# google/tfp-causalimpact

Measured on AMD Instinct MI355X. Metric: posterior samples/sec (T=1000, 10 covariates), higher is better.
Workload: dtype f32; 1 GPU; cfg2: T=1000, 10 covariates (P=11), LocalLinearTrend + spike-and-slab regression, Gibbs, W=112, S=1000; sampler=gibbs, chains_per_gpu=8, chains_total=8, parallelism=chains sharded over 1 GPU(s), no data-path collective, launcher=single process, collectives=none, ranks_seen=1

## Files before the change

tfp-causalimpact_amd/csrc/ci_kernels.h:

```cpp
#pragma once
#include <hip/hip_runtime.h>
#include <type_traits>
#include <stdint.h>

#include "ci_linalg.h"
#include "ci_rng.h"

namespace ci {

constexpr int NT = 256;
constexpr int NW = 4;
constexpr int MAXP = 52;
constexpr int HMC_MAXP = 128;

struct DevSeriesParams {
  double level_conc, level_scale, level_ub;
  double slope_conc, slope_scale, slope_ub;
  double obs_conc, obs_scale, obs_ub;
  double nonzero_prob;
  double init_level_loc, init_level_scale, init_slope_scale;
  double obs_scale0, level_scale0, slope_scale0;
  double n_obs;
};

struct KArgs {
  int T, P, W, S, C, B, chain_offset;
  int series_stream_base;
  uint32_t seed0, seed1;
  int x_in_lds;
  const float* y;
  const uint8_t* mask;
  const float* Xt;
  const double* xtx;
  const double* omega;
  const DevSeriesParams* sp;
  float* out_obs;
  float* out_level_scale;
  float* out_slope_scale;
  float* out_weights;
  float* out_level;
  float* out_slope;
  float* out_pred_mean;
  float* out_traj;
  long long* prof;
  unsigned int* progress;
  int progress_every;
  int dbg;
  const int* series_T;
  const int* series_ids;
};

__host__ __device__ inline uint32_t stream_mix32(uint32_t h) {
  h ^= h >> 16; h *= 0x85EBCA6Bu; h ^= h >> 13; h *= 0xC2B2AE35u; h ^= h >> 16;
  return h;
}
__host__ __device__ inline uint32_t stream_sid(int series_stream_base, int series) {
  return series_stream_base < 0 ? 0u : (uint32_t)(series_stream_base + series);
}
__host__ __device__ inline uint32_t stream_key0(uint32_t seed0, int series_stream_base, int series) {
  return seed0 ^ stream_mix32(stream_sid(series_stream_base, series));
}
__host__ __device__ inline uint32_t stream_key1(uint32_t seed1, int series_stream_base, int series) {
  return seed1 ^ stream_mix32(stream_sid(series_stream_base, series) * 0x9E3779B9u);
}

__device__ __forceinline__ void wave_sync() {
  __builtin_amdgcn_fence(__ATOMIC_SEQ_CST, "workgroup");
  __builtin_amdgcn_wave_barrier();
}

struct Prof {
  long long* p;
  long long t;
  __device__ __forceinline__ void start(long long* ptr, bool active) {
    p = active ? ptr : nullptr;
    if (p) t = clock64();
  }
  __device__ __forceinline__ void tick(int slot) {
    if (p) {
      const long long n = clock64();
      p[slot] += n - t;
      t = n;
    }
  }
};

struct NoProf {
  __device__ __forceinline__ void start(long long*, bool) {}
  __device__ __forceinline__ void tick(int) {}
};

template <class E> struct Arr { float f[sizeof(E) / 4]; };

template <class E> __device__ __forceinline__ E shfl_up_e(const E& e, int off) {
  Arr<E> a = __builtin_bit_cast(Arr<E>, e);
#pragma unroll
  for (int i = 0; i < (int)(sizeof(E) / 4); ++i) a.f[i] = __shfl_up(a.f[i], off, 64);
  return __builtin_bit_cast(E, a);
}
template <class E> __device__ __forceinline__ E shfl_down_e(const E& e, int off) {
  Arr<E> a = __builtin_bit_cast(Arr<E>, e);
#pragma unroll
  for (int i = 0; i < (int)(sizeof(E) / 4); ++i) a.f[i] = __shfl_down(a.f[i], off, 64);
  return __builtin_bit_cast(E, a);
}
template <class E> __device__ __forceinline__ void lds_store_e(float* p, const E& e) {
  const Arr<E> a = __builtin_bit_cast(Arr<E>, e);
#pragma unroll
  for (int i = 0; i < (int)(sizeof(E) / 4); ++i) p[i] = a.f[i];
}
template <class E> __device__ __forceinline__ E lds_load_e(const float* p) {
  Arr<E> a;
#pragma unroll
  for (int i = 0; i < (int)(sizeof(E) / 4); ++i) a.f[i] = p[i];
  return __builtin_bit_cast(E, a);
}

template <int CTRL, int ROW_MASK, class E> __device__ __forceinline__ E dpp_move_e(const E& e) {
  Arr<E> a = __builtin_bit_cast(Arr<E>, e);
#pragma unroll
  for (int i = 0; i < (int)(sizeof(E) / 4); ++i)
    a.f[i] = __int_as_float(__builtin_amdgcn_update_dpp(__float_as_int(a.f[i]), __float_as_int(a.f[i]),
                                                        CTRL, ROW_MASK, 0xF, false));
  return __builtin_bit_cast(E, a);
}
template <int CTRL, int ROW_MASK, class E> __device__ __forceinline__ E dpp_take_e(const E& e) {
  Arr<E> a = __builtin_bit_cast(Arr<E>, e);
#pragma unroll
  for (int i = 0; i < (int)(sizeof(E) / 4); ++i)
    a.f[i] = __int_as_float(__builtin_amdgcn_mov_dpp(__float_as_int(a.f[i]), CTRL, ROW_MASK, 0xF, true));
  return __builtin_bit_cast(E, a);
}
template <class E> __device__ __forceinline__ E select_e(bool c, const E& a, const E& b) {
  Arr<E> x = __builtin_bit_cast(Arr<E>, a);
  const Arr<E> y = __builtin_bit_cast(Arr<E>, b);
#pragma unroll
  for (int i = 0; i < (int)(sizeof(E) / 4); ++i) x.f[i] = c ? x.f[i] : y.f[i];
  return __builtin_bit_cast(E, x);
}

template <class E, class Op>
__device__ __forceinline__ E wave_scan_incl_fwd(const E& v, Op op, int lane) {
  E incl = v;
  const int r = lane & 15;
  { const E o = dpp_take_e<0x111, 0xF>(incl); if (r >= 1) incl = op(o, incl); }
  { const E o = dpp_take_e<0x112, 0xF>(incl); if (r >= 2) incl = op(o, incl); }
  { const E o = dpp_take_e<0x114, 0xF>(incl); if (r >= 4) incl = op(o, incl); }
  { const E o = dpp_take_e<0x118, 0xF>(incl); if (r >= 8) incl = op(o, incl); }
  { const E o = dpp_take_e<0x142, 0xA>(incl); if (lane & 16) incl = op(o, incl); }
  { const E o = dpp_take_e<0x143, 0xC>(incl); if (lane & 32) incl = op(o, incl); }
  return incl;
}
template <class E, class Op>
__device__ __forceinline__ E wave_scan_incl_bwd(const E& v, Op op, int lane) {
  E incl = v;
  const int r = lane & 15;
  { const E o = dpp_take_e<0x101, 0xF>(incl); if (r < 15) incl = op(incl, o); }
  { const E o = dpp_take_e<0x102, 0xF>(incl); if (r < 14) incl = op(incl, o); }
  { const E o = dpp_take_e<0x104, 0xF>(incl); if (r < 12) incl = op(incl, o); }
  { const E o = dpp_take_e<0x108, 0xF>(incl); if (r < 8) incl = op(incl, o); }
  {
    const Arr<E> b = __builtin_bit_cast(Arr<E>, dpp_take_e<0x150, 0xF>(incl));
    Arr<E> a;
#pragma unroll
    for (int i = 0; i < (int)(sizeof(E) / 4); ++i) {
      const auto s = __builtin_amdgcn_permlane16_swap((unsigned)__float_as_int(b.f[i]), 0u, false, false);
      a.f[i] = __int_as_float((int)s[1]);
    }
    const E o = __builtin_bit_cast(E, a);
    if ((lane & 16) == 0) incl = op(incl, o);
  }
  {
    Arr<E> a = __builtin_bit_cast(Arr<E>, incl);
#pragma unroll
    for (int i = 0; i < (int)(sizeof(E) / 4); ++i)
      a.f[i] = __int_as_float(__builtin_amdgcn_readlane(__float_as_int(a.f[i]), 32));
    const E o = __builtin_bit_cast(E, a);
    if ((lane & 32) == 0) incl = op(incl, o);
  }
  return incl;
}

template <class E, class Op>
__device__ __forceinline__ E block_scan_fwd_begin(const E& tot, Op op, float* slots, int lane, int wave) {
  constexpr int N = sizeof(E) / 4;
  const E incl = wave_scan_incl_fwd(tot, op, lane);
  if (lane == 63) lds_store_e(slots + wave * N, incl);
  return incl;
}
template <class E, class Op>
__device__ __forceinline__ E block_scan_fwd_finish(const E& incl, Op op, const E& ident, const float* slots,
                                                   int lane, int wave) {
  constexpr int N = sizeof(E) / 4;
  const E ex = select_e(lane == 0, ident, dpp_take_e<0x138, 0xF>(incl));
  if (wave == 0) return ex;
  E wp = lds_load_e<E>(slots);
  for (int ww = 1; ww < wave; ++ww) wp = op(wp, lds_load_e<E>(slots + ww * N));
  return op(wp, ex);
}
template <class E, class Op>
__device__ __forceinline__ E block_scan_excl_fwd(const E& tot, Op op, const E& ident, float* slots,
                                                 int lane, int wave) {
  const E incl = block_scan_fwd_begin(tot, op, slots, lane, wave);
  __syncthreads();
  return block_scan_fwd_finish(incl, op, ident, slots, lane, wave);
}

template <class E, class Op>
__device__ __forceinline__ E block_scan_excl_bwd(const E& tot, Op op, const E& ident, float* slots,
                                                 int lane, int wave) {
  constexpr int N = sizeof(E) / 4;
  const E incl = wave_scan_incl_bwd(tot, op, lane);
  if (lane == 0) lds_store_e(slots + wave * N, incl);
  __syncthreads();
  const E ex = select_e(lane == 63, ident, dpp_take_e<0x130, 0xF>(incl));
  if (wave == NW - 1) return ex;
  E ws = lds_load_e<E>(slots + (wave + 1) * N);
  for (int ww = wave + 2; ww < NW; ++ww) ws = op(ws, lds_load_e<E>(slots + ww * N));
  return op(ex, ws);
}

template <int L>
__device__ __forceinline__ void global_row_load_wide(const float* __restrict__ row, int t0, int T,
                                                     float (&v)[L]) {
  static_assert(L % 4 == 0, "wide rows need L % 4 == 0");
#pragma unroll
  for (int q = 0; q < L / 4; ++q) {
    const int t = t0 + 4 * q;
    const float4 x = *reinterpret_cast<const float4*>(row + (t < T ? t : T - 4));
    const bool in = t < T;
    v[4 * q] = in ? x.x : 0.f; v[4 * q + 1] = in ? x.y : 0.f;
    v[4 * q + 2] = in ? x.z : 0.f; v[4 * q + 3] = in ? x.w : 0.f;
  }
}
template <int L>
__device__ __forceinline__ void global_row_load_scalar(const float* __restrict__ row, int t0, int T,
                                                       float (&v)[L]) {
#pragma unroll
  for (int l = 0; l < L; ++l) {
    const int t = t0 + l;
    const float x = row[t < T ? t : T - 1];
    v[l] = t < T ? x : 0.f;
// ... 3079 lines not shown
```

tfp-causalimpact_amd/csrc/ci_kernels8.h:

```cpp
#pragma once
#include "ci_kernels.h"

namespace ci {

constexpr int SCHED_DEFAULT = (2 << 4) | (1 << 6) | (0 << 8) | (2 << 10) | (2 << 12) | (0 << 14);
constexpr int NT8 = 512;
constexpr int NW8 = 8;
constexpr int PRE_MAXS = 16;

struct PreTables {
  double* tsw;
  double* V;
  double* rdk;
  double* hand;
};
constexpr size_t PRE_HALF_DOUBLES = PRE_MAXS * 16 + 16 * 16 + 16;
__host__ __device__ constexpr size_t pre_tables_bytes() {
  return sizeof(double) * (2 * PRE_HALF_DOUBLES + 20) + 16;
}
__device__ __forceinline__ PreTables pre_tables_at(unsigned char* base, int parity) {
  PreTables tb;
  double* d = (double*)base + (size_t)(parity & 1) * PRE_HALF_DOUBLES;
  tb.tsw = d; d += PRE_MAXS * 16;
  tb.V = d; d += 16 * 16;
  tb.rdk = d;
  tb.hand = (double*)base + 2 * PRE_HALF_DOUBLES;
  return tb;
}
constexpr int HAND_SCALE = 16, HAND_INTS = 17;

struct PreState {
  double c[4];
  double diag;
  double rdk;
  unsigned long long S;
  int n_sw;
  int valid;
};

template <int CTRL> __device__ __forceinline__ double dpp_ror_add_d(double v) {
  const int lo = __builtin_amdgcn_update_dpp(0, __double2loint(v), CTRL, 0xF, 0xF, false);
  const int hi = __builtin_amdgcn_update_dpp(0, __double2hiint(v), CTRL, 0xF, 0xF, false);
  return v + __hiloint2double(hi, lo);
}
__device__ __forceinline__ double row_sum16_d(double v) {
  v = dpp_ror_add_d<0x128>(v);
  v = dpp_ror_add_d<0x124>(v);
  v = dpp_ror_add_d<0x122>(v);
  v = dpp_ror_add_d<0x121>(v);
  return readlane_d(v, 0);
}

template <int KR>
__device__ __forceinline__ void sweep_rec_kr(QCols& m, int k, int lane, double& t_out, double& rd_out) {
  const int kq = k >> 2, j = lane & 15, q = lane >> 4;
  const double ckr = m.c[KR];
  const double rd = fast_rcp(readlane_d(ckr, k + 16 * kq));
  const double rowk = bperm_d(ckr, j + 16 * kq);
  const bool isk = j == k;
  const double t = isk ? 1.0 : rowk * rd;
  double colk[4];
#pragma unroll
  for (int r = 0; r < 4; ++r) colk[r] = bperm_d(m.c[r], k + 16 * q);
  __builtin_amdgcn_sched_barrier(0);
#pragma unroll
  for (int r = 0; r < 4; ++r) m.c[r] = isk ? colk[r] * rd : m.c[r] - colk[r] * t;
  m.c[KR] = (q == kq) ? (isk ? -rd : t) : m.c[KR];
  m.diag = isk ? -rd : m.diag - rowk * rowk * rd;
  t_out = t;
  rd_out = rd;
}
__device__ __forceinline__ void sweep_rec(QCols& m, int k, int lane, double& t_out, double& rd_out) {
  switch (k & 3) {
    case 0: sweep_rec_kr<0>(m, k, lane, t_out, rd_out); break;
    case 1: sweep_rec_kr<1>(m, k, lane, t_out, rd_out); break;
    case 2: sweep_rec_kr<2>(m, k, lane, t_out, rd_out); break;
    default: sweep_rec_kr<3>(m, k, lane, t_out, rd_out); break;
  }
}

struct PreRun {
  QCols m;
  double rdk;
  unsigned long long pending;
  int n;
  int phase;
};
__device__ __forceinline__ void pre_begin(PreRun& st, unsigned long long S) {
  st.pending = S;
  st.n = 0;
  st.rdk = 0.0;
  st.phase = 0;
}
__device__ __forceinline__ void pre_step(PreRun& st, const RegLds& R, int P, double var_next,
                                         unsigned long long S, int lane, const PreTables& tb,
                                         PreState& ps) {
  const int j = lane & 15, q = lane >> 4;
  const bool live = j < P;
  const int col = live ? j : 0;
  if (st.phase == 0) {
#pragma unroll
    for (int r = 0; r < 4; ++r) {
      const int i = 4 * q + r;
      double om = 0.0, xx = 0.0;
      if (live && i < P) {
        om = R.omega[i * P + col];
        xx = R.xtx[i * P + col];
      }
      st.m.c[r] = om * var_next + xx;
      st.m.p[r] = 0.0;
    }
    st.m.diag = live ? R.omega[col * P + col] * var_next + R.xtx[col * P + col] : 1.0;
    st.m.cb = 0.0; st.m.corner = 0.0; st.m.pdiag = 0.0;
    st.phase = st.pending != 0ull ? 1 : 2;
  } else if (st.phase == 1) {
    const int k = __builtin_amdgcn_readfirstlane(__ffsll((long long)st.pending) - 1);
    double t, rd;
    sweep_rec(st.m, k, lane, t, rd);
    if (q == 0) tb.tsw[st.n * 16 + j] = t;
    st.rdk = (j == k) ? rd : st.rdk;
    ++st.n;
    st.pending &= st.pending - 1ull;
    if (st.pending == 0ull) st.phase = 2;
  } else {
#pragma unroll
    for (int r = 0; r < 4; ++r) tb.V[(4 * q + r) * 16 + j] = st.m.c[r];
    if (q == 0) tb.rdk[j] = st.rdk;
    ps.n_sw = st.n;
#pragma unroll
    for (int r = 0; r < 4; ++r) ps.c[r] = st.m.c[r];
    ps.diag = st.m.diag;
    ps.rdk = st.rdk;
    ps.S = S;
    ps.valid = 1;
    st.phase = 3;
  }
}

__device__ __forceinline__ void weights_backsub(const PreTables& tb, const double* pre, int P,
                                                unsigned long long S, double mean, double new_scale,
                                                int lane, float* w) {
  const int j = lane & 15, q = lane >> 4;
  const bool live = j < P;
  const float zf = reinterpret_cast<const float*>(pre + 24)[live ? j : 0];
  const bool inS = ((S >> j) & 1ull) != 0ull;
  const int pos = __popcll(S & ((1ull << j) - 1ull));
  const int n_sw = __popcll(S);
  const double rsz = (double)__fsqrt_rn((float)tb.rdk[j]) * (double)zf;
  double tt[PRE_MAXS];
#pragma unroll
  for (int s = 0; s < PRE_MAXS; ++s) tt[s] = tb.tsw[s * 16 + j];
  double u = 0.0;
#pragma unroll
  for (int s = PRE_MAXS - 1; s >= 0; --s) {
    if (s < n_sw) {
      double dot = (inS && pos > s) ? tt[s] * u : 0.0;
      dot = dpp_ror_add_d<0x128>(dot);
      dot = dpp_ror_add_d<0x124>(dot);
      dot = dpp_ror_add_d<0x122>(dot);
      dot = dpp_ror_add_d<0x121>(dot);
      u = (inS && pos == s) ? rsz - dot : u;
    }
  }
  if (q == 0 && live) w[j] = inS ? (float)(mean + new_scale * u) : 0.f;
}

template <class PF, class Pub>
__device__ __forceinline__ double spike_slab_draw_pre(const RegLds& R, int P,
                                                      const DevSeriesParams& sp,
                                                      double prev_obs_scale, double g_obs,
                                                      int lane, PriorCarry& pc, const double* pre,
                                                      const PreTables& tb, const PreState& ps,
                                                      const float* red, PF& prof, Pub publish) {
  const double prev_var = prev_obs_scale * prev_obs_scale;
  const double a_post = sp.obs_conc + 0.5 * sp.n_obs;
  const bool all_in = sp.nonzero_prob >= 1.0;
  const int j = lane & 15, q = lane >> 4;
  const bool live = j < P;
  const int col = live ? j : 0;
  QCols m;
#pragma unroll
  for (int r = 0; r < 4; ++r) { m.c[r] = ps.c[r]; m.p[r] = pc.p[r]; }
  m.diag = ps.diag;
  m.pdiag = pc.pdiag;
  m.cb = live ? (double)red[col] : 0.0;
  m.corner = (double)red[RED_YTY];
  unsigned long long S = ps.S;
  {
    double v[16], bk[16];
#pragma unroll
    for (int g = 0; g < 4; ++g) {
      if (4 * g < P) {
#pragma unroll
        for (int k = 4 * g; k < 4 * g + 4; ++k) {
          v[k] = tb.V[k * 16 + j];
          bk[k] = (double)red[k];
        }
      } else {
#pragma unroll
        for (int k = 4 * g; k < 4 * g + 4; ++k) { v[k] = 0.0; bk[k] = 0.0; }
      }
    }
    double acc0 = 0.0, acc1 = 0.0;
#pragma unroll
    for (int k = 0; k < 16; k += 2) {
      acc0 = ((S >> k) & 1ull) ? fma(v[k], bk[k], acc0) : acc0;
      acc1 = ((S >> (k + 1)) & 1ull) ? fma(v[k + 1], bk[k + 1], acc1) : acc1;
    }
    const bool inj = ((S >> j) & 1ull) != 0ull;
    const double bj = m.cb;
    m.cb = live ? (inj ? 0.0 : bj) - (acc0 + acc1) : 0.0;
    m.corner -= row_sum16_d((live && inj) ? bj * m.cb : 0.0);
  }
  prof.tick(21);
  bool dirty = false;
  if (!all_in) {
    const int rank = reinterpret_cast<const int*>(pre + 16)[j];
    const double uflip = pre[j];
    const double logit_pi =
        (double)(__logf((float)sp.nonzero_prob) - __logf((float)(1.0 - sp.nonzero_prob)));
    int s_cur = 0;
    const double inv_prev_var = fast_rcp(prev_var);
    for (;;) {
      const bool in = ((S >> j) & 1ull) != 0ull;
      const double sg = in ? -1.0 : 1.0;
      const double rap = fast_rcp(sg * m.diag);
      const double beta_old = sp.obs_scale + 0.5 * m.corner;
      const double x = -0.5 * sg * m.cb * m.cb * rap * fast_rcp(beta_old);
      const double pscale = in ? inv_prev_var : prev_var;
      const double delta = 0.5 * (double)__logf((float)(sg * m.pdiag * pscale * rap)) +
                           sg * logit_pi - (a_post - 1.0) * fast_log1p(x);
      const float prob = 1.0f / (1.0f + __expf(-(float)delta));
      const bool acc = live && q == 0 && rank >= s_cur && uflip < (double)prob;
      unsigned long long cand = __ballot(acc);
      if (cand == 0ull) break;
      int best = -1, best_rank = 1 << 20;
      for (; cand != 0ull; cand &= cand - 1ull) {
        const int jj = __ffsll((long long)cand) - 1;
        const int rj = __builtin_amdgcn_readlane(rank, jj);
        if (rj < best_rank) { best_rank = rj; best = jj; }
      }
      best = __builtin_amdgcn_readfirstlane(best);
      sweep_q<true>(m, best, ((S >> best) & 1ull) != 0ull, lane);
      S ^= 1ull << best;
      s_cur = best_rank + 1;
      dirty = true;
    }
  }
  prof.tick(22);
#pragma unroll
  for (int r = 0; r < 4; ++r) pc.p[r] = m.p[r];
  pc.pdiag = m.pdiag;
  pc.S = S;
  pc.valid = 1;
  const double beta_post = sp.obs_scale + 0.5 * m.corner;
  double var = beta_post * fast_rcp(g_obs);
  if (var > sp.obs_ub) var = sp.obs_ub;
  const double new_scale = (double)__fsqrt_rn((float)var);
  const double mean = m.cb;
  if (publish(new_scale, mean, S, !dirty)) {
    prof.tick(23);
    return new_scale;
  }
  if (!dirty) {
    weights_backsub(tb, pre, P, S, mean, new_scale, lane, R.w);
  } else {
    const float zf = reinterpret_cast<const float*>(pre + 24)[col];
    double mu = 0.0, umine = 0.0;
    for (unsigned long long mm = S; mm != 0ull;) {
      const int aidx = __builtin_amdgcn_readfirstlane(63 - __clzll((long long)mm));
      mm &= ~(1ull << aidx);
      const double vaa = -readlane_d(m.diag, aidx);
      const double mua = readlane_d(mu, aidx);
      const double za = (double)__int_as_float(__builtin_amdgcn_readlane(__float_as_int(zf), aidx));
      const double ua = mua + (double)__fsqrt_rn((float)vaa) * za;
      const double t = unsweep_q(m, aidx, lane);
      if (j == aidx) umine = ua; else mu += t * (ua - mua);
    }
    if (q == 0 && live) R.w[j] = ((S >> j) & 1ull) ? (float)(mean + new_scale * umine) : 0.f;
  }
  wave_sync();
  prof.tick(23);
  return new_scale;
}


template <int D, int L> struct Lay8 {
  static constexpr size_t TP = (size_t)NT * L;
  static constexpr size_t a16(size_t x) { return (x + 15) & ~(size_t)15; }
  static constexpr size_t off_ctx = 0;
  static constexpr size_t off_xtx = a16(sizeof(SerialCtx));
  static constexpr size_t off_omega = off_xtx + 16 * 16 * sizeof(double);
  static constexpr size_t off_bvec = off_omega + 16 * 16 * sizeof(double);
  static constexpr size_t off_w = off_bvec + a16(20 * sizeof(double));
  static constexpr size_t off_scal = off_w + 16 * sizeof(float);
  static constexpr size_t off_red = off_scal + 32 * sizeof(float);
  static constexpr size_t off_slots = off_red + 32 * sizeof(float);
  static constexpr size_t off_xlast = off_slots + 3 * NW * 16 * sizeof(float);
  static constexpr size_t off_gam = off_xlast + a16((size_t)NT * D * sizeof(float));
  static constexpr size_t off_pre = off_gam + a16((8 + 64 + 4) * sizeof(double));
  static constexpr size_t off_tgv = off_pre + a16(pre_tables_bytes());
  static constexpr size_t off_z = off_tgv + TP * sizeof(float);
  static constexpr bool PARK = L >= 8;
  static constexpr size_t off_xw = off_z + 3 * TP * sizeof(float);
  static constexpr size_t off_y = off_xw + (PARK ? TP * sizeof(float) : 0);
  static constexpr size_t off_x = off_y + (PARK ? TP * sizeof(float) : 0);
  static __host__ __device__ constexpr size_t total(int P) { return off_x + (size_t)P * TP * sizeof(float); }
};
enum Scal8 { SC8_INIT_LOC = 8, SC8_INIT_VAR = 9, SC8_INIT_SVAR = 10, SC8_ZINIT = 12 };

template <int D, int L, bool PROF = false, bool XG = false>
__global__ __launch_bounds__(NT8) void gibbs_kernel8(KArgs a) {
  using PF = typename std::conditional<PROF, Prof, NoProf>::type;
  using LY = Lay8<D, L>;
  extern __shared__ __attribute__((aligned(16))) unsigned char smem[];
  const int tid = threadIdx.x, lane = tid & 63;
  const int wave = __builtin_amdgcn_readfirstlane(tid >> 6);
  const int series = blockIdx.x / a.C, chain = blockIdx.x % a.C;
  const int T = a.T, P = a.P;
  constexpr int TPAD = NT * L;
  SerialCtx* cx = (SerialCtx*)(smem + LY::off_ctx);
  float* scal = (float*)(smem + LY::off_scal);
  float* red = (float*)(smem + LY::off_red);
  float* slots = (float*)(smem + LY::off_slots);
  float* xlast = (float*)(smem + LY::off_xlast);
  float* wls = (float*)(smem + LY::off_w);
  float* tgv = (float*)(smem + LY::off_tgv);
  float* zb = (float*)(smem + LY::off_z);
  float* xwb = (float*)(smem + LY::off_xw);
  float* ybuf = (float*)(smem + LY::off_y);
  double* gam = (double*)(smem + LY::off_gam);
  const size_t chain_lin = (size_t)series * a.C + chain;
  const int n_iter = a.W + a.S;

  Rng rng;
  rng.k0 = stream_key0(a.seed0, a.series_stream_base, series);
  rng.k1 = stream_key1(a.seed1, a.series_stream_base, series);
  rng.chain = (uint32_t)(a.chain_offset + chain);

  const float* yg = a.y + (size_t)series * T;
  const uint8_t* mg = a.mask + (size_t)series * T;
  const float* Xg = a.Xt + (size_t)series * P * T;
  const float* Xs = XG ? Xg : (const float*)(smem + LY::off_x);
  const bool xwide = L % 4 == 0 && (T & 3) == 0 && (reinterpret_cast<uintptr_t>(Xg) & 15) == 0;
  RegLds R;
  R.xtx = (double*)(smem + LY::off_xtx);
  R.omega = (double*)(smem + LY::off_omega);
  R.aug[0] = R.aug[1] = R.pri[0] = R.pri[1] = R.chol = R.zv = R.uperm = nullptr;
  R.nz = R.perm = R.idx = nullptr;
  R.bvec = (double*)(smem + LY::off_bvec);
  R.w = wls;
  if (tid == 0) {
    cx->sp = a.sp[series];
    cx->obs_scale = cx->sp.obs_scale0;
    cx->level_scale = cx->sp.level_scale0;
    cx->slope_scale = cx->sp.slope_scale0;
    cx->R = R;
    cx->scal = scal;
    cx->red = red;
    cx->out_obs = a.out_obs;
    cx->out_level_scale = a.out_level_scale;
    cx->out_slope_scale = a.out_slope_scale;
    cx->out_weights = a.out_weights;
    cx->chain_lin = chain_lin;
    cx->rng = rng;
    cx->P = P; cx->T = T; cx->D = D; cx->W = a.W; cx->S = a.S; cx->n_iter = n_iter;
    cx->prof = nullptr;
    scal[SC_OBS_DK] = (float)cx->sp.obs_scale0;
    scal[SC8_INIT_LOC] = (float)cx->sp.init_level_loc;
    scal[SC8_INIT_VAR] = (float)(cx->sp.init_level_scale * cx->sp.init_level_scale);
    scal[SC8_INIT_SVAR] = (float)(cx->sp.init_slope_scale * cx->sp.init_slope_scale);
  }
  {
    for (int e = tid; e < P * P; e += NT8) {
      R.xtx[e] = a.xtx[(size_t)series * P * P + e];
      R.omega[e] = a.omega[(size_t)series * P * P + e];
    }
    if constexpr (!XG) {
      float* xw_ = (float*)(smem + LY::off_x);
      for (int j = 0; j < P; ++j)
        for (int t = tid; t < TPAD; t += NT8) xw_[j * TPAD + t] = (t < T) ? Xg[(size_t)j * T + t] : 0.f;
    }
    if (tid < 16) wls[tid] = 0.f;
  }
  __syncthreads();
  unsigned char* pre_base = smem + LY::off_pre;

  if (wave > NW) {
    const int e = wave - NW - 1;
    constexpr int NTASK = (D == 2) ? 3 : 2;
    constexpr int ROUNDS = NTASK * L;
    constexpr int N0 = ROUNDS / 3, N1 = (ROUNDS - N0) / 2;
    const int k_lo = e == 0 ? 0 : (e == 1 ? N0 : N0 + N1);
    const int k_hi = e == 0 ? N0 : (e == 1 ? N0 + N1 : ROUNDS);
    const int n_my = k_hi - k_lo;
    PF eprof;
    eprof.start(a.prof, a.prof != nullptr && blockIdx.x == 0 && wave == NW + 1 && lane == 0);
    auto normals_round = [&](int k, uint32_t it_for) __attribute__((always_inline)) {
      const int task = k / L, blk = k - task * L;
      const int slot = (D == 2) ? task : (task == 0 ? 0 : 2);
      const uint32_t site = slot == 0 ? SITE_PRIOR_LEVEL : (slot == 1 ? SITE_PRIOR_SLOPE : SITE_PRIOR_OBS);
      const int c = 64 * blk + lane;
      const U4 r = site_call(rng, it_for, site, 0, (uint32_t)c);
      float z[4];
      normals4(r, z);
      *reinterpret_cast<float4*>(zb + (size_t)slot * TPAD + 4 * c) = make_float4(z[0], z[1], z[2], z[3]);
    };
    auto role_work = [&](int it_next) __attribute__((always_inline)) {
      if (it_next > n_iter) return;
      if (e == 0) {
        serial_gammas<1>(cx, it_next, lane, gam + 4 * (it_next & 1));
      } else if (e == 1) {
        if (it_next < n_iter) spike_slab_randoms(rng, (uint32_t)it_next, P, lane, gam + 8 + 32 * (it_next & 1));
      } else if (it_next < n_iter) {
        float zi[1];
        fill_normals<1>(rng, (uint32_t)it_next, SITE_PRIOR_INIT, 0, (uint32_t)lane, zi);
        asm volatile("" : "+v"(zi[0]));
        if (lane < D) scal[SC8_ZINIT + 2 * (it_next & 1) + lane] = zi[0];
      }
    };
    role_work(0);
    for (int k = k_lo; k < k_hi; ++k) normals_round(k, 0u);
    eprof.tick(30);
    const int sched = (a.dbg & 0xFFFF) ? (a.dbg & 0xFFFF) : SCHED_DEFAULT;
    const int mode = sched & 3;
    const int scale = L >= 4 ? L / 4 : 1;
    const int c_3 = e == 2 ? 0 : ((sched >> 10) & 3) * scale, c_4 = ((sched >> 12) & 3) * scale,
              c_a = ((sched >> 14) & 3) * scale;
    const int r_3 = mode == 1 ? n_my : (mode == 2 ? 0 : (c_3 < n_my ? c_3 : n_my));
    const int r_4 = mode == 1 ? n_my : (mode == 2 ? 0 : (r_3 + c_4 < n_my ? r_3 + c_4 : n_my));
    const int r_5 = mode == 2 ? 0 : (n_my - c_a > r_4 ? n_my - c_a : r_4);
    for (int it = 0; it <= n_iter; ++it) {
      __syncthreads();
      eprof.tick(31);
      xt_sums_wave<L, 2, XG>(tgv, Xs, TPAD, P, 2 * wave, wave == NW8 - 1, red, lane, T, xwide);
      eprof.tick(30);
      __syncthreads();
      eprof.tick(31);
      role_work(it + 1);
      eprof.tick(30);
      __syncthreads();
      eprof.tick(31);
      if (e == 2 && it < n_iter) {
        const PreTables tb = pre_tables_at(pre_base, it);
        const int* hi_ = reinterpret_cast<const int*>(tb.hand + HAND_INTS);
        if (hi_[2] != 0) {
          const unsigned long long S = ((unsigned long long)(unsigned)hi_[1] << 32) | (unsigned)hi_[0];
          weights_backsub(tb, gam + 8 + 32 * (it & 1), P, S, tb.hand[lane & 15], tb.hand[HAND_SCALE],
                          lane, wls);
        }
      }
      int r = 0;
      if (it < n_iter)
        for (; r < r_3; ++r) normals_round(k_lo + r, (uint32_t)(it + 1));
      eprof.tick(30);
      __syncthreads();
      eprof.tick(31);
      if (it == n_iter) break;
      for (; r < r_4; ++r) normals_round(k_lo + r, (uint32_t)(it + 1));
      eprof.tick(30);
      __syncthreads();
      eprof.tick(31);
      for (; r < r_5; ++r) normals_round(k_lo + r, (uint32_t)(it + 1));
      eprof.tick(30);
      __syncthreads();
      eprof.tick(31);
      for (; r < n_my; ++r) normals_round(k_lo + r, (uint32_t)(it + 1));
      eprof.tick(30);
    }
    return;
  }

  if (wave == NW) {
    PriorCarry pc;
    pc.valid = 0; pc.S = 0ull; pc.pdiag = 0.0;
#pragma unroll
    for (int r = 0; r < 4; ++r) pc.p[r] = 0.0;
    PreState ps;
    ps.valid = 0; ps.S = 0ull; ps.n_sw = 0; ps.diag = 1.0; ps.rdk = 0.0;
#pragma unroll
    for (int r = 0; r < 4; ++r) ps.c[r] = 0.0;
    PF rprof;
    rprof.start(a.prof, a.prof != nullptr && blockIdx.x == 0 && lane == 0);
    double obs_scale = cx->sp.obs_scale0, level_scale = cx->sp.level_scale0, slope_scale = cx->sp.slope_scale0;
    const DevSeriesParams sp = cx->sp;
    float* o_obs = a.out_obs;
    float* o_ls = a.out_level_scale;
    float* o_ss = a.out_slope_scale;
    float* o_w = a.out_weights;
    const int sched = (a.dbg & 0xFFFF) ? (a.dbg & 0xFFFF) : SCHED_DEFAULT;
    const int mode = sched & 3;
    for (int it = 0; it <= n_iter; ++it) {
      __syncthreads();
      __builtin_amdgcn_s_setprio(3);
      xt_sums_wave<L, 2, XG>(tgv, Xs, TPAD, P, 2 * wave, false, red, lane, T, xwide);
      __syncthreads();
      rprof.tick(16);
      const PreTables tb = pre_tables_at(pre_base, it);
      if (lane < P + 1) R.bvec[lane] = (double)red[lane < P ? lane : RED_YTY];
      const float wprev = lane < P ? wls[lane] : 0.f;
      const double* gm = gam + 4 * (it & 1);
      const double g_level = gm[0], g_slope = gm[1], g_obs = gm[2];
      const double emit_obs = obs_scale;
      rprof.tick(20);
      auto publish4 = [&](double ns, double mean, unsigned long long S, bool clean) __attribute__((always_inline)) {
        if (lane == 0) scal[SC_OBS_DK] = (float)ns;
        if (lane < 16) tb.hand[lane] = mean;
        if (lane == 0) {
          tb.hand[HAND_SCALE] = ns;
          int* hi_ = reinterpret_cast<int*>(tb.hand + HAND_INTS);
          hi_[0] = (int)(unsigned)(S & 0xFFFFFFFFull);
          hi_[1] = (int)(unsigned)(S >> 32);
          hi_[2] = clean ? 1 : 0;
        }
        rprof.tick(22);
        __builtin_amdgcn_s_setprio(0);
        __syncthreads();
        rprof.tick(18);
        return clean;
      };
      auto publish1 = [&](double ns) __attribute__((always_inline)) { (void)publish4(ns, 0.0, 0ull, false); };
      if (it < n_iter) {
        if (ps.valid && ps.S == pc.S) {
          obs_scale = spike_slab_draw_pre(R, P, sp, obs_scale, g_obs, lane, pc, gam + 8 + 32 * (it & 1), tb,
                                          ps, red, rprof, publish4);
        } else {
          NoProf np;
          wave_sync();
          obs_scale = spike_slab_draw_regs(R, P, sp, obs_scale, g_obs, rng, (uint32_t)it, lane, np, pc,
                                           gam + 8 + 32 * (it & 1), publish1);
        }
      } else {
        publish1(obs_scale);
      }
      rprof.tick(23);
      auto after_b3 = [&]() __attribute__((always_inline)) {
        if (it > 0) {
          auto clipped_scale = [](double scale, double ss, double g, double ub) {
            const double s = (double)__fsqrt_rn((float)((scale + 0.5 * ss) * fast_rcp(g)));
            return s < ub ? s : ub;
          };
          double ssl = 0.0, sss = 0.0;
#pragma unroll
          for (int w = 0; w < NW; ++w) {
            ssl += (double)red[RED_INC + 2 * w];
            sss += (double)red[RED_INC + 2 * w + 1];
          }
          level_scale = clipped_scale(sp.level_scale, ssl, g_level, sp.level_ub);
          if (D == 2) slope_scale = clipped_scale(sp.slope_scale, sss, g_slope, sp.slope_ub);
          const int s = it - 1 - a.W;
          if (s >= 0) {
            const size_t o = chain_lin * a.S + s;
            if (lane == 0) {
              if (o_obs) o_obs[o] = (float)emit_obs;
              if (o_ls) o_ls[o] = (float)level_scale;
              if (o_ss) o_ss[o] = (float)(D == 2 ? slope_scale : 0.0);
            }
            if (o_w && lane < P) o_w[o * P + lane] = wprev;
          }
        }
      };
      if (it == n_iter) {
        __syncthreads();
        after_b3();
        break;
      }
      const PreTables tbn = pre_tables_at(pre_base, it + 1);
      const double var_next = obs_scale * obs_scale;
      PreRun st;
      pre_begin(st, pc.S);
      const int n_sw = __popcll(pc.S);
      const int p_3 = (sched >> 4) & 3, p_4 = (sched >> 6) & 3, p_a = (sched >> 8) & 3;
      const int s_3 = mode == 1 ? n_sw + 2 : (mode == 2 ? 0 : 1 + (p_3 < n_sw ? p_3 : n_sw));
      const int s_4 = mode == 1 ? n_sw + 2 : (mode == 2 ? 0 : (s_3 + p_4 < 1 + n_sw ? s_3 + p_4 : 1 + n_sw));
      const int s_5 = mode == 1 ? n_sw + 2 : (mode == 2 ? 0 : (1 + n_sw - p_a > s_4 ? 1 + n_sw - p_a : s_4));
      int step = 0;
      for (; st.phase != 3 && step < s_3; ++step) pre_step(st, R, P, var_next, pc.S, lane, tbn, ps);
      rprof.tick(19);
      __syncthreads();
      rprof.tick(17);
      after_b3();
      for (; st.phase != 3 && step < s_4; ++step) pre_step(st, R, P, var_next, pc.S, lane, tbn, ps);
      rprof.tick(19);
      __syncthreads();
      rprof.tick(29);
      for (; st.phase != 3 && step < s_5; ++step) pre_step(st, R, P, var_next, pc.S, lane, tbn, ps);
      rprof.tick(19);
      __syncthreads();
      rprof.tick(29);
      for (; st.phase != 3; ++step) pre_step(st, R, P, var_next, pc.S, lane, tbn, ps);
      rprof.tick(19);
    }
    return;
  }

  __builtin_amdgcn_s_setprio(1);
  const int t0 = tid * L;
  float yv[L];
  uint32_t maskbits = 0;
#pragma unroll
  for (int l = 0; l < L; ++l) {
    const int t = t0 + l;
    const bool in = t < T;
    yv[l] = in ? yg[t] : 0.f;
    const bool m = in ? (mg[t] != 0) : true;
    if (m) { maskbits |= (1u << l); yv[l] = 0.f; }
  }
  if constexpr (LY::PARK) store_targets<L>(ybuf, t0, yv);
  const float init_loc = scal[SC8_INIT_LOC], init_var = scal[SC8_INIT_VAR], init_svar = scal[SC8_INIT_SVAR];
  const DevSeriesParams* spp = &cx->sp;
  const double sp_level_scale0 = spp->level_scale0, sp_slope_scale0 = spp->slope_scale0;
  const double sp_level_scale = spp->level_scale, sp_slope_scale = spp->slope_scale;
  const double sp_level_ub = spp->level_ub, sp_slope_ub = spp->slope_ub;
  float lev[L], slp[L], xw[L], pm_acc[L];
#pragma unroll
  for (int l = 0; l < L; ++l) { lev[l] = 0.f; slp[l] = 0.f; xw[l] = 0.f; pm_acc[l] = 0.f; }
  float* o_level = a.out_level ? a.out_level + chain_lin * a.S * T : nullptr;
  float* o_slope = a.out_slope ? a.out_slope + chain_lin * a.S * T : nullptr;
  float* o_traj = a.out_traj ? a.out_traj + chain_lin * a.S * T : nullptr;
  PF prof;
  prof.start(a.prof, a.prof != nullptr && blockIdx.x == 0 && tid == 0);
  for (int it = 0; it <= n_iter; ++it) {
    {
      float tg[L], yq[L];
      if constexpr (LY::PARK) {
        lds_row_load<L>(ybuf + t0, yq);
      } else {
#pragma unroll
        for (int l = 0; l < L; ++l) yq[l] = yv[l];
      }
#pragma unroll
      for (int l = 0; l < L; ++l) {
        const bool obs = ((maskbits >> l) & 1u) == 0u;
        tg[l] = obs ? (yq[l] - lev[l]) : 0.f;
      }
      store_targets<L>(tgv, t0, tg);
      xlast[tid * D] = lev[L - 1];
      if constexpr (D == 2) xlast[tid * D + 1] = slp[L - 1];
    }
    __syncthreads();
    xt_sums_wave<L, 2, XG>(tgv, Xs, TPAD, P, 2 * wave, false, red, lane, T, xwide);
    {
      float ssl = 0.f, sss = 0.f;
      float pl = (tid > 0) ? xlast[(tid - 1) * D] : 0.f;
      float ps_ = 0.f;
      if constexpr (D == 2) ps_ = (tid > 0) ? xlast[(tid - 1) * D + 1] : 0.f;
#pragma unroll
      for (int l = 0; l < L; ++l) {
        const int t = t0 + l;
        if (t >= 1 && t < T) {
          float dl = lev[l] - pl;
          if constexpr (D == 2) {
            dl -= ps_;
            const float ds = slp[l] - ps_;
            sss = fmaf(ds, ds, sss);
          }
          ssl = fmaf(dl, dl, ssl);
        }
        pl = lev[l];
        if constexpr (D == 2) ps_ = slp[l];
      }
      const float s1 = wave_prefix_dpp(ssl), s2 = wave_prefix_dpp(sss);
      if (lane == 63) {
        red[RED_INC + 2 * wave] = s1;
        red[RED_INC + 2 * wave + 1] = s2;
      }
    }
    const float so_prev = scal[SC_OBS_DK];
    __syncthreads();
    prof.tick(0);

    float zl[L], zs[L], zo[L];
    const float* zit = zb + t0;
    lds_row_load<L>(zit, zl);
    if constexpr (D == 2) {
      lds_row_load<L>(zit + TPAD, zs);
    } else {
#pragma unroll
      for (int l = 0; l < L; ++l) zs[l] = 0.f;
    }
    lds_row_load<L>(zit + 2 * TPAD, zo);
    if (it > a.W) {
      const int s = it - 1 - a.W;
      float zp[L];
      fill_normals<L>(rng, (uint32_t)(it - 1), SITE_PRED, 0, (uint32_t)t0, zp);
      float tr[L];
      if constexpr (LY::PARK) {
        float xwp[L], acc[L];
        lds_row_load<L>(xwb + t0, xwp);
        float* pm = a.out_pred_mean ? a.out_pred_mean + chain_lin * T : nullptr;
        const bool vec = (T & 3) == 0;
        if (pm != nullptr && s > 0) {
          if (vec) {
#pragma unroll
            for (int q = 0; q < L / 4; ++q) {
              const int t = t0 + 4 * q;
              const float4 v = t < T ? *(const float4*)(pm + t) : make_float4(0.f, 0.f, 0.f, 0.f);
              acc[4 * q] = v.x; acc[4 * q + 1] = v.y; acc[4 * q + 2] = v.z; acc[4 * q + 3] = v.w;
            }
          } else {
#pragma unroll
            for (int l = 0; l < L; ++l) acc[l] = t0 + l < T ? pm[t0 + l] : 0.f;
          }
        } else {
#pragma unroll
          for (int l = 0; l < L; ++l) acc[l] = 0.f;
        }
#pragma unroll
        for (int l = 0; l < L; ++l) {
          const float loc = lev[l] + xwp[l];
          acc[l] += loc;
          tr[l] = fmaf(so_prev, zp[l], loc);
        }
        if (pm != nullptr) {
          if (vec) {
#pragma unroll
            for (int q = 0; q < L / 4; ++q) {
              const int t = t0 + 4 * q;
              if (t < T) *(float4*)(pm + t) = make_float4(acc[4 * q], acc[4 * q + 1], acc[4 * q + 2], acc[4 * q + 3]);
            }
          } else {
#pragma unroll
            for (int l = 0; l < L; ++l)
              if (t0 + l < T) pm[t0 + l] = acc[l];
          }
        }
      } else {
#pragma unroll
        for (int l = 0; l < L; ++l) {
          const float loc = lev[l] + xw[l];
          pm_acc[l] += loc;
          tr[l] = fmaf(so_prev, zp[l], loc);
        }
      }
      const size_t row = (size_t)s * T;
      bool vec_done = false;
      if constexpr (L % 4 == 0) {
        if ((T & 3) == 0) {
          vec_done = true;
#pragma unroll
          for (int q = 0; q < L / 4; ++q) {
            const int t = t0 + 4 * q;
            if (t < T) {
              if (o_level) *(float4*)(o_level + row + t) = make_float4(lev[4 * q], lev[4 * q + 1], lev[4 * q + 2], lev[4 * q + 3]);
              if (o_slope) *(float4*)(o_slope + row + t) = make_float4(slp[4 * q], slp[4 * q + 1], slp[4 * q + 2], slp[4 * q + 3]);
              if (o_traj) *(float4*)(o_traj + row + t) = make_float4(tr[4 * q], tr[4 * q + 1], tr[4 * q + 2], tr[4 * q + 3]);
            }
          }
        }
      }
      if (!vec_done) {
#pragma unroll
        for (int l = 0; l < L; ++l) {
          const int t = t0 + l;
          if (t < T) {
            if (o_level) o_level[row + t] = lev[l];
            if (o_slope) o_slope[row + t] = slp[l];
            if (o_traj) o_traj[row + t] = tr[l];
          }
        }
      }
    }
    Vec<D> sig;
    PElem<D> pincl = pelem_identity<D>();
    {
      auto clipped_scale = [](double scale, double ss, double g, double ub) {
        const double s = (double)__fsqrt_rn((float)((scale + 0.5 * ss) * fast_rcp(g)));
        return s < ub ? s : ub;
      };
      double level_scale = sp_level_scale0, slope_scale = sp_slope_scale0;
      if (it > 0) {
        const double* gm = gam + 4 * (it & 1);
        double ssl = 0.0, sss = 0.0;
#pragma unroll
        for (int w = 0; w < NW; ++w) {
          ssl += (double)red[RED_INC + 2 * w];
          sss += (double)red[RED_INC + 2 * w + 1];
        }
        level_scale = clipped_scale(sp_level_scale, ssl, gm[0], sp_level_ub);
        if constexpr (D == 2) slope_scale = clipped_scale(sp_slope_scale, sss, gm[1], sp_slope_ub);
      }
      sig.v[0] = (float)level_scale;
      if constexpr (D == 2) sig.v[1] = (float)slope_scale;
      if (it < n_iter) pincl = dk_prior_begin<D, L>(sig, zl, zs, slots, lane, wave);
    }
    const bool publish = a.progress != nullptr && it > a.W &&
                         ((it - a.W) % a.progress_every == 0 || it - a.W == a.S);
    if (publish) asm volatile("s_waitcnt vmcnt(0)" ::: "memory");
    prof.tick(2);
    __syncthreads();
    prof.tick(1);
    if (publish) {
      if (tid == 0) {
        __builtin_amdgcn_fence(__ATOMIC_RELEASE, "");
        asm volatile("s_waitcnt vmcnt(0)" ::: "memory");
        __hip_atomic_store(a.progress + chain_lin, (unsigned int)(it - a.W), __ATOMIC_RELAXED,
                           __HIP_MEMORY_SCOPE_SYSTEM);
      }
    }
    if (it == n_iter) {
      __syncthreads();
      break;
    }

    DkModel<D> md;
    {
      const float so = scal[SC_OBS_DK];
      md.H = so * so;
      md.sig = sig;
      md.a1 = vzero<D>();
      md.a1.v[0] = init_loc;
      md.p1.v[0] = init_var;
      if constexpr (D == 2) md.p1.v[1] = init_svar;
    }
    Vec<D> q;
#pragma unroll
    for (int i = 0; i < D; ++i) q.v[i] = md.sig.v[i] * md.sig.v[i];
    const PElem<D> ppre = dk_prior_finish<D>(pincl, slots, lane, wave);
    const FMElem<D> fme = dk_matrix_chunk<D, L>(md, q, maskbits, tid);
    const FMElem<D> mincl = dk_matrix_scan_begin<D>(fme, slots + NW * 16, lane, wave);
    prof.tick(24);
    __syncthreads();
    float Pin[D * (D + 1) / 2];
    dk_matrix_scan_finish<D>(mincl, slots + NW * 16, lane, wave, Pin);
    DkMats<D, L> km;
    dk_matrix_local<D, L>(md, q, maskbits, tid, Pin, km);
    prof.tick(25);

    float resid[L];
#pragma unroll
    for (int l = 0; l < L; ++l) xw[l] = 0.f;
    {
      float wv[16];
      lds_row_load<16>(wls, wv);
      if constexpr (!XG) {
#pragma unroll
        for (int j = 0; j < 16; ++j) {
          const int jj = j < P ? j : P - 1;
          const float wj = j < P ? wv[j] : 0.f;
          float xr[L];
          lds_row_load<L>(Xs + jj * TPAD + t0, xr);
#pragma unroll
          for (int l = 0; l < L; ++l) xw[l] = fmaf(xr[l], wj, xw[l]);
        }
      } else {
        constexpr int RB = L >= 16 ? 2 : (L >= 8 ? 4 : 8);
        auto stream = [&](auto load_row) __attribute__((always_inline)) {
          unsigned long long todo = __ballot(lane < P && wls[lane < P ? lane : 0] != 0.f);
          while (todo != 0ull) {
            float xr[RB][L], wj[RB];
#pragma unroll
            for (int u = 0; u < RB; ++u) {
              const bool have = todo != 0ull;
              const int j = have ? __ffsll((long long)todo) - 1 : 0;
              todo &= todo - 1ull;
              wj[u] = have ? wls[j] : 0.f;
              load_row(j, xr[u]);
            }
#pragma unroll
            for (int u = 0; u < RB; ++u)
#pragma unroll
              for (int l = 0; l < L; ++l) xw[l] = fmaf(xr[u][l], wj[u], xw[l]);
          }
        };
        if (xwide) {
          if constexpr (L % 4 == 0)
            stream([&](int j, float (&xr)[L]) { global_row_load_wide<L>(Xg + (size_t)j * T, t0, T, xr); });
        } else {
          stream([&](int j, float (&xr)[L]) { global_row_load_scalar<L>(Xg + (size_t)j * T, t0, T, xr); });
        }
      }
    }
    if constexpr (LY::PARK) {
      float yq[L];
      lds_row_load<L>(ybuf + t0, yq);
#pragma unroll
      for (int l = 0; l < L; ++l) resid[l] = yq[l] - xw[l];
    } else {
#pragma unroll
      for (int l = 0; l < L; ++l) resid[l] = yv[l] - xw[l];
    }
    if constexpr (LY::PARK) store_targets<L>(xwb, t0, xw);
    const Vec<D> a1e = dk_initial_mean<D>(md, rng, (uint32_t)it, tid, scal + SC8_ZINIT + 2 * (it & 1));
    Vec<D> xp[L];
    float ytil[L];
    dk_prior_path<D, L>(md, ppre, resid, zl, zs, zo, xp, ytil);
    prof.tick(3);
    const AElem<D> fe = dk_fwd_chunk<D, L>(km, a1e, ytil, maskbits, tid);
    const AElem<D> fincl = aff_fwd_begin<D>(fe, slots, lane, wave);
    prof.tick(27);
    __syncthreads();
    const Vec<D> mf = aff_fwd_finish<D>(fincl, slots, lane, wave);
    prof.tick(5);
    Vec<D> ap[L];
    float vf[L];
    const AElem<D> be = dk_fwd_local_bwd_chunk<D, L>(km, a1e, ytil, maskbits, tid, mf, ap, vf);
    const AElem<D> bincl = aff_bwd_begin<D>(be, slots + 2 * NW * 16, lane, wave);
    prof.tick(6);
    __syncthreads();
    const Vec<D> rr = aff_bwd_finish<D>(bincl, slots + 2 * NW * 16, lane, wave);
    prof.tick(28);
    Vec<D> x[L];
    dk_bwd_fixup<D, L>(km, rr, ap, vf, xp, x);
#pragma unroll
    for (int l = 0; l < L; ++l) {
      lev[l] = x[l].v[0];
      if constexpr (D == 2) slp[l] = x[l].v[1];
    }
    prof.tick(7);
  }

  if (a.out_pred_mean) {
    const float inv = 1.0f / (float)(a.S > 0 ? a.S : 1);
    float* pm = a.out_pred_mean + chain_lin * T;
#pragma unroll
    for (int l = 0; l < L; ++l) {
      const int t = t0 + l;
      if constexpr (LY::PARK) {
        if (t < T) pm[t] = (a.S > 0 ? pm[t] : 0.f) * inv;
      } else {
        if (t < T) pm[t] = pm_acc[l] * inv;
      }
    }
  }
}

}
```

Measured before the change: 1.171 million posterior samples/sec.

## Split spike-slab RHS dot across half-waves and hoist obs-scale reciprocal and logit

For small L and P>8, V is stored interleaved as double2 so each half-wave computes half the masked dot product with vector loads, and the halves are recombined with permlane32_swap. The gamma loads, obs reciprocal and logit(pi) are hoisted out of the per-iteration critical path, and the bvec LDS writes are deferred to the fallback path. Role work also gets a raised wave priority for small L. Extra profiling marks are added, but they compile away under NoProf. The layout change adds a split code path and applies only to certain L/P combinations.

New measurement: 1.188 million posterior samples/sec (median of 6 runs). 1.01x the previous value.

```diff
diff --git a/tfp-causalimpact_amd/csrc/ci_kernels.h b/tfp-causalimpact_amd/csrc/ci_kernels.h
--- a/tfp-causalimpact_amd/csrc/ci_kernels.h
+++ b/tfp-causalimpact_amd/csrc/ci_kernels.h
@@ -83,11 +83,15 @@
       t = n;
     }
   }
+  __device__ __forceinline__ void mark() {
+    if (p) t = clock64();
+  }
 };
 
 struct NoProf {
   __device__ __forceinline__ void start(long long*, bool) {}
   __device__ __forceinline__ void tick(int) {}
+  __device__ __forceinline__ void mark() {}
 };
 
 template <class E> struct Arr { float f[sizeof(E) / 4]; };
diff --git a/tfp-causalimpact_amd/csrc/ci_kernels8.h b/tfp-causalimpact_amd/csrc/ci_kernels8.h
--- a/tfp-causalimpact_amd/csrc/ci_kernels8.h
+++ b/tfp-causalimpact_amd/csrc/ci_kernels8.h
@@ -50,6 +50,15 @@
   v = dpp_ror_add_d<0x121>(v);
   return readlane_d(v, 0);
 }
+__device__ __forceinline__ void halves_d(double v, double& of_lower, double& of_upper) {
+  const unsigned lo = (unsigned)__double2loint(v), hi = (unsigned)__double2hiint(v);
+  const auto sl = __builtin_amdgcn_permlane32_swap(lo, lo, false, false);
+  const auto sh = __builtin_amdgcn_permlane32_swap(hi, hi, false, false);
+  of_lower = __hiloint2double((int)sh[0], (int)sl[0]);
+  of_upper = __hiloint2double((int)sh[1], (int)sl[1]);
+}
+
+template <int L> __device__ __forceinline__ bool rhs_split(int P) { return L <= 4 && P > 8; }
 
 template <int KR>
 __device__ __forceinline__ void sweep_rec_kr(QCols& m, int k, int lane, double& t_out, double& rd_out) {
@@ -94,7 +103,7 @@
 }
 __device__ __forceinline__ void pre_step(PreRun& st, const RegLds& R, int P, double var_next,
                                          unsigned long long S, int lane, const PreTables& tb,
-                                         PreState& ps) {
+                                         PreState& ps, bool split) {
   const int j = lane & 15, q = lane >> 4;
   const bool live = j < P;
   const int col = live ? j : 0;
@@ -123,8 +132,14 @@
     st.pending &= st.pending - 1ull;
     if (st.pending == 0ull) st.phase = 2;
   } else {
-#pragma unroll
-    for (int r = 0; r < 4; ++r) tb.V[(4 * q + r) * 16 + j] = st.m.c[r];
+    if (split) {
+      double2* V2 = reinterpret_cast<double2*>(tb.V);
+      V2[q * 16 + j] = make_double2(st.m.c[0], st.m.c[2]);
+      V2[(4 + q) * 16 + j] = make_double2(st.m.c[1], st.m.c[3]);
+    } else {
+#pragma unroll
+      for (int r = 0; r < 4; ++r) tb.V[(4 * q + r) * 16 + j] = st.m.c[r];
+    }
     if (q == 0) tb.rdk[j] = st.rdk;
     ps.n_sw = st.n;
 #pragma unroll
@@ -165,13 +180,15 @@
   if (q == 0 && live) w[j] = inS ? (float)(mean + new_scale * u) : 0.f;
 }
 
-template <class PF, class Pub>
+template <bool HOIST, class PF, class Pub>
 __device__ __forceinline__ double spike_slab_draw_pre(const RegLds& R, int P,
                                                       const DevSeriesParams& sp,
                                                       double prev_obs_scale, double g_obs,
-                                                      int lane, PriorCarry& pc, const double* pre,
-                                                      const PreTables& tb, const PreState& ps,
-                                                      const float* red, PF& prof, Pub publish) {
+                                                      double rg_obs_early, double logit_pi_early,
+                                                      bool split, int lane, PriorCarry& pc,
+                                                      const double* pre, const PreTables& tb,
+                                                      const PreState& ps, const float* red, PF& prof,
+                                                      Pub publish) {
   const double prev_var = prev_obs_scale * prev_obs_scale;
   const double a_post = sp.obs_conc + 0.5 * sp.n_obs;
   const bool all_in = sp.nonzero_prob >= 1.0;
@@ -187,25 +204,57 @@
   m.corner = (double)red[RED_YTY];
   unsigned long long S = ps.S;
   {
-    double v[16], bk[16];
-#pragma unroll
-    for (int g = 0; g < 4; ++g) {
-      if (4 * g < P) {
-#pragma unroll
-        for (int k = 4 * g; k < 4 * g + 4; ++k) {
-          v[k] = tb.V[k * 16 + j];
-          bk[k] = (double)red[k];
-        }
-      } else {
-#pragma unroll
-        for (int k = 4 * g; k < 4 * g + 4; ++k) { v[k] = 0.0; bk[k] = 0.0; }
-      }
-    }
     double acc0 = 0.0, acc1 = 0.0;
-#pragma unroll
-    for (int k = 0; k < 16; k += 2) {
-      acc0 = ((S >> k) & 1ull) ? fma(v[k], bk[k], acc0) : acc0;
-      acc1 = ((S >> (k + 1)) & 1ull) ? fma(v[k + 1], bk[k + 1], acc1) : acc1;
+    if (split) {
+      const int h = q >> 1;
+      const double2* V2 = reinterpret_cast<const double2*>(tb.V) + h * 64 + j;
+      const float4* b4 = reinterpret_cast<const float4*>(red);
+      double2 v[4];
+      float4 f[4];
+#pragma unroll
+      for (int g = 0; g < 4; ++g) {
+        if (4 * g < P) {
+          v[g] = V2[g * 16];
+          f[g] = b4[g];
+        } else {
+          v[g] = make_double2(0.0, 0.0);
+          f[g] = make_float4(0.f, 0.f, 0.f, 0.f);
+        }
+      }
+      double ba[4], bb[4];
+#pragma unroll
+      for (int g = 0; g < 4; ++g) {
+        ba[g] = (double)(h ? f[g].y : f[g].x);
+        bb[g] = (double)(h ? f[g].w : f[g].z);
+      }
+      const unsigned Sh = (unsigned)(S & 0xFFFFull) >> h;
+      double acc = 0.0;
+#pragma unroll
+      for (int g = 0; g < 4; ++g) {
+        acc = ((Sh >> (4 * g)) & 1u) ? fma(v[g].x, ba[g], acc) : acc;
+        acc = ((Sh >> (4 * g + 2)) & 1u) ? fma(v[g].y, bb[g], acc) : acc;
+      }
+      halves_d(acc, acc0, acc1);
+    } else {
+      double v[16], bk[16];
+#pragma unroll
+      for (int g = 0; g < 4; ++g) {
+        if (4 * g < P) {
+#pragma unroll
+          for (int k = 4 * g; k < 4 * g + 4; ++k) {
+            v[k] = tb.V[k * 16 + j];
+            bk[k] = (double)red[k];
+          }
+        } else {
+#pragma unroll
+          for (int k = 4 * g; k < 4 * g + 4; ++k) { v[k] = 0.0; bk[k] = 0.0; }
+        }
+      }
+#pragma unroll
+      for (int k = 0; k < 16; k += 2) {
+        acc0 = ((S >> k) & 1ull) ? fma(v[k], bk[k], acc0) : acc0;
+        acc1 = ((S >> (k + 1)) & 1ull) ? fma(v[k + 1], bk[k + 1], acc1) : acc1;
+      }
     }
     const bool inj = ((S >> j) & 1ull) != 0ull;
     const double bj = m.cb;
@@ -217,8 +266,9 @@
   if (!all_in) {
     const int rank = reinterpret_cast<const int*>(pre + 16)[j];
     const double uflip = pre[j];
-    const double logit_pi =
-        (double)(__logf((float)sp.nonzero_prob) - __logf((float)(1.0 - sp.nonzero_prob)));
+    double logit_pi = logit_pi_early;
+    if constexpr (!HOIST)
+      logit_pi = (double)(__logf((float)sp.nonzero_prob) - __logf((float)(1.0 - sp.nonzero_prob)));
     int s_cur = 0;
     const double inv_prev_var = fast_rcp(prev_var);
     for (;;) {
@@ -254,7 +304,7 @@
   pc.S = S;
   pc.valid = 1;
   const double beta_post = sp.obs_scale + 0.5 * m.corner;
-  double var = beta_post * fast_rcp(g_obs);
+  double var = beta_post * (HOIST ? rg_obs_early : fast_rcp(g_obs));
   if (var > sp.obs_ub) var = sp.obs_ub;
   const double new_scale = (double)__fsqrt_rn((float)var);
   const double mean = m.cb;
@@ -396,6 +446,8 @@
     const int n_my = k_hi - k_lo;
     PF eprof;
     eprof.start(a.prof, a.prof != nullptr && blockIdx.x == 0 && wave == NW + 1 && lane == 0);
+    PF aprof;
+    aprof.start(a.prof, a.prof != nullptr && blockIdx.x == 0 && lane == 0);
     auto normals_round = [&](int k, uint32_t it_for) __attribute__((always_inline)) {
       const int task = k / L, blk = k - task * L;
       const int slot = (D == 2) ? task : (task == 0 ? 0 : 2);
@@ -437,8 +489,12 @@
       eprof.tick(30);
       __syncthreads();
       eprof.tick(31);
+      aprof.mark();
+      if constexpr (L <= 4) __builtin_amdgcn_s_setprio(2);
       role_work(it + 1);
+      if constexpr (L <= 4) __builtin_amdgcn_s_setprio(0);
       eprof.tick(30);
+      aprof.tick(11 + e);
       __syncthreads();
       eprof.tick(31);
       if (e == 2 && it < n_iter) {
@@ -490,17 +546,29 @@
     float* o_w = a.out_weights;
     const int sched = (a.dbg & 0xFFFF) ? (a.dbg & 0xFFFF) : SCHED_DEFAULT;
     const int mode = sched & 3;
+    constexpr bool HOIST = L <= 4;
+    const bool split = rhs_split<L>(P);
+    double logit_pi = 0.0;
+    if constexpr (HOIST)
+      logit_pi = (double)(__logf((float)sp.nonzero_prob) - __logf((float)(1.0 - sp.nonzero_prob)));
     for (int it = 0; it <= n_iter; ++it) {
       __syncthreads();
       __builtin_amdgcn_s_setprio(3);
       xt_sums_wave<L, 2, XG>(tgv, Xs, TPAD, P, 2 * wave, false, red, lane, T, xwide);
+      const double* gm = gam + 4 * (it & 1);
+      double g_level, g_slope, g_obs, rg_obs = 0.0;
+      if constexpr (HOIST) {
+        g_level = gm[0]; g_slope = gm[1]; g_obs = gm[2];
+        rg_obs = fast_rcp(g_obs);
+        asm volatile("" : "+v"(rg_obs));
+      }
       __syncthreads();
       rprof.tick(16);
       const PreTables tb = pre_tables_at(pre_base, it);
-      if (lane < P + 1) R.bvec[lane] = (double)red[lane < P ? lane : RED_YTY];
+      if constexpr (!HOIST)
+        if (lane < P + 1) R.bvec[lane] = (double)red[lane < P ? lane : RED_YTY];
       const float wprev = lane < P ? wls[lane] : 0.f;
-      const double* gm = gam + 4 * (it & 1);
-      const double g_level = gm[0], g_slope = gm[1], g_obs = gm[2];
+      if constexpr (!HOIST) { g_level = gm[0]; g_slope = gm[1]; g_obs = gm[2]; }
       const double emit_obs = obs_scale;
       rprof.tick(20);
       auto publish4 = [&](double ns, double mean, unsigned long long S, bool clean) __attribute__((always_inline)) {
@@ -522,10 +590,12 @@
       auto publish1 = [&](double ns) __attribute__((always_inline)) { (void)publish4(ns, 0.0, 0ull, false); };
       if (it < n_iter) {
         if (ps.valid && ps.S == pc.S) {
-          obs_scale = spike_slab_draw_pre(R, P, sp, obs_scale, g_obs, lane, pc, gam + 8 + 32 * (it & 1), tb,
-                                          ps, red, rprof, publish4);
+          obs_scale = spike_slab_draw_pre<HOIST>(R, P, sp, obs_scale, g_obs, rg_obs, logit_pi, split, lane,
+                                                 pc, gam + 8 + 32 * (it & 1), tb, ps, red, rprof, publish4);
         } else {
           NoProf np;
+          if constexpr (HOIST)
+            if (lane < P + 1) R.bvec[lane] = (double)red[lane < P ? lane : RED_YTY];
           wave_sync();
           obs_scale = spike_slab_draw_regs(R, P, sp, obs_scale, g_obs, rng, (uint32_t)it, lane, np, pc,
                                            gam + 8 + 32 * (it & 1), publish1);
@@ -575,20 +645,20 @@
       const int s_4 = mode == 1 ? n_sw + 2 : (mode == 2 ? 0 : (s_3 + p_4 < 1 + n_sw ? s_3 + p_4 : 1 + n_sw));
       const int s_5 = mode == 1 ? n_sw + 2 : (mode == 2 ? 0 : (1 + n_sw - p_a > s_4 ? 1 + n_sw - p_a : s_4));
       int step = 0;
-      for (; st.phase != 3 && step < s_3; ++step) pre_step(st, R, P, var_next, pc.S, lane, tbn, ps);
+      for (; st.phase != 3 && step < s_3; ++step) pre_step(st, R, P, var_next, pc.S, lane, tbn, ps, split);
       rprof.tick(19);
       __syncthreads();
       rprof.tick(17);
       after_b3();
-      for (; st.phase != 3 && step < s_4; ++step) pre_step(st, R, P, var_next, pc.S, lane, tbn, ps);
+      for (; st.phase != 3 && step < s_4; ++step) pre_step(st, R, P, var_next, pc.S, lane, tbn, ps, split);
       rprof.tick(19);
       __syncthreads();
       rprof.tick(29);
-      for (; st.phase != 3 && step < s_5; ++step) pre_step(st, R, P, var_next, pc.S, lane, tbn, ps);
+      for (; st.phase != 3 && step < s_5; ++step) pre_step(st, R, P, var_next, pc.S, lane, tbn, ps, split);
       rprof.tick(19);
       __syncthreads();
       rprof.tick(29);
-      for (; st.phase != 3; ++step) pre_step(st, R, P, var_next, pc.S, lane, tbn, ps);
+      for (; st.phase != 3; ++step) pre_step(st, R, P, var_next, pc.S, lane, tbn, ps, split);
       rprof.tick(19);
     }
     return;
@@ -620,6 +690,8 @@
   float* o_traj = a.out_traj ? a.out_traj + chain_lin * a.S * T : nullptr;
   PF prof;
   prof.start(a.prof, a.prof != nullptr && blockIdx.x == 0 && tid == 0);
+  PF aprof;
+  aprof.start(a.prof, a.prof != nullptr && blockIdx.x == 0 && wave > 0 && lane == 0);
   for (int it = 0; it <= n_iter; ++it) {
     {
       float tg[L], yq[L];
@@ -669,6 +741,7 @@
     const float so_prev = scal[SC_OBS_DK];
     __syncthreads();
     prof.tick(0);
+    aprof.mark();
 
     float zl[L], zs[L], zo[L];
     const float* zit = zb + t0;
@@ -788,6 +861,7 @@
                          ((it - a.W) % a.progress_every == 0 || it - a.W == a.S);
     if (publish) asm volatile("s_waitcnt vmcnt(0)" ::: "memory");
     prof.tick(2);
+    aprof.tick(7 + wave);
     __syncthreads();
     prof.tick(1);
     if (publish) {
```
